# esteinig/scrubby

Hardware: AMD Instinct MI355X
Metric: reads/s depleted (2x150bp PE vs CHM13v2-sized reference), records classified per second (higher is better)
Workload: dtype u64/i32 (f32 in the chain gap penalty)

## Files before the change

scrubby_amd/csrc/sh_classify.hip:

```cpp
#include "sh_common.h"
#include "sh_wave.h"
#include "sh_merge4.h"
#include "sh_sketch.h"
#include "sh_chain.h"
#include "sh_long.h"
#include "sh_ctx_layout.h"
#include <algorithm>
#include <chrono>
#include <memory>

#define SH_SPLIT ((sh_status)-2)
#define K1_LIST_CAP 8
#define K2_CAP 32
#define DP_SMALL_CAP 32
#define SORT_LDS_A 512
#define SORT_LDS_B 2048
#define SORT_LDS_C 4096
#define N_SORT_CLS 6
#define SORT_CLS_GIANT 5
#define GT 2048u
#define LOCUS_N0 1024u
#define LOCUS_N1 4096u
#define LOCUS_MAX_N 65535u
#define LOCUS_RUN_MAX 16

__device__ inline uint32_t lane_id() { return threadIdx.x & 63; }

struct Counters {
    uint32_t n_small, n_resketch, n_big[2], n_big_defer[2], n_defer, n_small2;
    uint32_t n_big_total, pad1;
    uint32_t n_sort[N_SORT_CLS], n_giant_tiles, n_giant_passes;
    uint32_t expand_ticket, lc_ticket;
    uint32_t top_ticket[N_SORT_CLS];
    uint32_t sort_ticket[N_SORT_CLS];
    uint32_t n_long_segs, pad2;
    uint32_t ext_reason[8];
    uint32_t lext_exact_direct, lext_pad_d;
    uint32_t lc_why[16]; unsigned long long lc_anchors[16];
    uint32_t ext_overflow, ext_n_list, ext_ticket, ext_regions, ext_dropped, ext_n_redo, ext_n_list2, ext_ticket2, ext_n_redo2, ext_ticket3, ext_n_unres, ext_ticket_unres, ext_n_unres_in, ext_pad8;
    uint32_t ext_n_recs[SINK_SHARDS]; unsigned long long ext_n_anch[SINK_SHARDS];
    uint32_t lext_n_exact2, lext_ticket_exact2;
    uint32_t lext_hist[64]; uint32_t lext_ticket_g, lext_pad3; uint32_t lext_n_big, lext_ticket_big, lext_n_big2, lext_ticket_big2, lext_ticket_b, lext_pad2, lext_rechained, lext_rmq_tie, lext_err_read, lext_unresolved, lext_err_code, lext_pad;
    unsigned long long lext_clk[LR_NCLK], lext_d[8], lext_slow, lext_kernel_sum;
    uint32_t n_cl[4], cl_ticket, cl_ticket3;
    uint32_t n_leg_reason[4];
    uint32_t pair_mid[4];
    unsigned long long arena_cursor, anchor_cursor;
    unsigned long long cl_tot[4], cl_anchor_tot[4], cl_dbg[10], pf_dbg[16];
    unsigned long long sort_tot[N_SORT_CLS + 1], sort_anchor_tot[N_SORT_CLS + 1];
    unsigned long long sh_mini[64], sh_anchors[64];
    uint32_t sh_host[64], sh_clusters[64], sh_pair[64];
    uint32_t sh_late[64], sh_deferred[64];
    uint32_t sh_pf_reads[64], sh_pf_dirty[64], sh_top[64];
    uint32_t sh_lemma[64];
    uint32_t n_locus[3], locus_ticket[3], lr_n_fb, lr_locus_reads; unsigned long long lr_locus_in, lr_locus_kept;
    uint32_t lr_fb_why[8], lr_fb_had, lr_pad, lr_probe_why[8];
    uint32_t lext_n_unres, lext_ticket_unres, lext_n_unres_in, lext_pad4, lext_n_exact, lext_ticket_exact, lext_rmq_open, lext_pad5;
    unsigned long long ext_clk[8], ext_diag[8]; uint32_t ext_hist[24];
    unsigned long long lext_slow2, lext_slow3, lext_slow_part[4], lext_sum_part[4], lext_clk_big[LR_NCLK], lext_d_big[8], lext_phase_max[LR_NCLK];
    uint32_t lext_started, lext_t0_done;
    unsigned long long stage_cursor;
};
#define SHARD() ((blockIdx.x + (blockIdx.x >> 6)) & 63)

struct WaveAlloc {
    uint32_t cur = 0, end = 0;
    __device__ inline uint32_t take(uint32_t *counter, uint32_t n, uint32_t chunk, uint32_t &lo, uint32_t &hi)
    {
        lo = hi = 0;
        if (cur + n > end) {
            lo = cur; hi = end;
            const uint32_t want = n > chunk ? n : chunk;
            uint32_t base = 0;
            if (lane_id() == 0) base = atomicAdd(counter, want);
            base = (uint32_t)__builtin_amdgcn_readfirstlane((int)base);
            cur = base; end = base + want;
        }
        const uint32_t r = cur;
        cur += n;
        return r;
    }
};

__device__ inline uint32_t prefix_popc(uint64_t mask)
{
    return __builtin_amdgcn_mbcnt_hi((uint32_t)(mask >> 32), __builtin_amdgcn_mbcnt_lo((uint32_t)mask, 0u));
}
__device__ inline uint32_t wave_append(uint32_t *counter, bool pred)
{
    uint64_t mask = __ballot(pred);
    if (mask == 0) return ~0u;
    uint32_t base = 0;
    uint32_t leader = __ffsll((unsigned long long)mask) - 1;
    if (lane_id() == leader) base = atomicAdd(counter, (uint32_t)__popcll(mask));
    base = (uint32_t)wave_bcast((int32_t)base, (int)leader);
    return pred ? base + prefix_popc(mask) : ~0u;
}

__device__ inline void write_trace(sh_trace *tr, uint64_t r, int32_t n_mini, int32_t n_seed, int32_t n_anchor, int32_t rep_len,
                                   int32_t rechained, int32_t n_chain, int32_t best, int32_t flag)
{
    if (!tr) return;
    int4 *p = (int4 *)(tr + r);
    p[0] = make_int4(n_mini, n_seed, n_anchor, rep_len);
    p[1] = make_int4(rechained, n_chain, best, flag);
    p[2] = make_int4(0, 0, 0, 0);
}

struct K1Args {
    const uint8_t *bases; const uint64_t *offsets; uint64_t n_reads, n_bases;
    const uint4 *slots; uint32_t lg_slots; int32_t k;
    uint4 *records; uint32_t seed_cap;
    uint32_t *k1info; uint8_t *flags; sh_trace *trace;
    uint32_t *work_small, *work_resketch, *work_big; Counters *ctr;
// ... 1472 lines not shown
        if (in_lds) {
            uint64_t x = lane < n_a ? e_x[lane] : ~0ull;
            uint32_t q = lane < n_a ? e_q[lane] : 0u;
            uint64_t xp = wave_shr1_u64(x, 0ull);
            if (__ballot(lane > 0 && lane < n_a && x < xp) != 0) {
                wave_rank_sort(x, q, n_a, lane);
                __syncthreads();
                if (lane < n_a) { e_x[lane] = x; e_q[lane] = q; }
                __syncthreads();
            }
            int32_t n_u = 0, best = 0;
            bool lemma_done = false;
            if (a.t_mode && P.ext_lemma) {
                BestChain bc{};
                chain_sorted<false>(e_x, e_q, e_f, e_pt, n_a, lane, 64, qlen, P, nullptr, BigList{e_bstart, e_blen, &e_bcount, 8}, n_u, best, n_clusters,
                                    nullptr, nullptr, nullptr, r, nullptr, &bc, region_hash(qlen), -1, TandemQ{recb, n_seed, 1u, qlen, LONG ? 1u : info >> 31});
                unsigned long long zmax = bc.n ? bc.z : 0ull;
                zmax = wave_all_max_u64(zmax);
                const uint64_t holders = __ballot(bc.n > 0 && bc.z == zmax);
                const uint64_t any = __ballot(bc.n > 0);
                bool ok = false;
                if (any == 0) ok = true;
                else if (__popcll(holders) == 1) {
                    int32_t code = 0;
                    MidReq mid{0, 0, 0, 0, 0};
                    if (bc.n > 0 && bc.z == zmax && !bc.tie) {
                        SliceStore S{(const uint64_t *)&e_x[bc.base], (const uint32_t *)&e_q[bc.base], e_f + bc.base, e_pt + 2 * (size_t)bc.base};
                        code = chain_lemma(S, bc.zi, bc.end_i, P, (uint32_t)(S.X(bc.zi) >> 32), mid);
                    }
                    const bool mid_ok = resolve_mid_wave(code == 2, mid, a.BC.bases + a.offsets[r], qlen, a.BC, P);
                    ok = __ballot(code == 1 || (code == 2 && mid_ok)) != 0;
                }
                lemma_done = ok;
                if (ok && any != 0) ++n_lemma;
                if (!ok) { n_u = 0; best = 0; __syncthreads(); }
            }
            if (!lemma_done)
            chain_sorted<false>(e_x, e_q, e_f, e_pt, n_a, lane, 64, qlen, P, nullptr, BigList{e_bstart, e_blen, &e_bcount, 8}, n_u, best, n_clusters,
                                nullptr, nullptr, a.emit ? &sink_l : nullptr, r, nullptr);
            n_u = wave_all_add(n_u); best = wave_all_max(best);
            if (lane == 0) { a.B.acc_nu[w] = n_u; a.B.acc_best[w] = best; }
            if ((a.dbg & DBG_STATS) && lane == 0) { atomicAdd(&a.ctr->sort_tot[N_SORT_CLS], 1ull); atomicAdd(&a.ctr->sort_anchor_tot[N_SORT_CLS], (unsigned long long)n_a); }
            __syncthreads();
        } else if (to_stage) {
            const int lc = n_a <= LOCUS_N0 ? 0 : (n_a <= LOCUS_N1 ? 1 : 2);
            if (lane == 0) { const uint32_t li = atomicAdd(&a.ctr->n_locus[lc], 1u); SortItem it{w, n_a, (uint32_t)qlen, 0, off}; a.locus_items[lc][li] = it; }
        } else {
            uint32_t lo, hi;
            const uint32_t si = al_sort[cls].take(&a.ctr->n_sort[cls], 1, cls <= 1 ? 32u : (cls <= 3 ? 8u : 1u), lo, hi);
            SortItem *const items = a.B.tabs->sort_items[cls];
            for (uint32_t i = lo + lane; i < hi; i += 64) items[i].n = 0;
            if (lane == 0) { SortItem it{w, n_a, (uint32_t)qlen, late ? late_item(r, n_seed) : 0u, off}; items[si] = it; }
            n_late += late;
            if ((a.dbg & DBG_STATS) && lane == 0) { atomicAdd(&a.ctr->sort_tot[cls], 1ull); atomicAdd(&a.ctr->sort_anchor_tot[cls], (unsigned long long)n_a); }
        }
    }
    for (int cls = 0; cls < N_SORT_CLS; ++cls)
        for (uint32_t i = al_sort[cls].cur + lane; i < al_sort[cls].end; i += 64) a.B.tabs->sort_items[cls][i].n = 0;
    if (lane == 0 && anchors_wave) atomicAdd(&a.ctr->sh_anchors[SHARD()], anchors_wave);
    n_clusters = wave_sum_u32(n_clusters);
    if (lane == 0 && n_clusters) atomicAdd(&a.ctr->sh_clusters[SHARD()], n_clusters);
    if (lane == 0 && n_pair) atomicAdd(&a.ctr->sh_pair[SHARD()], n_pair);
    if (lane == 0 && n_late && !a.quiet) atomicAdd(&a.ctr->sh_late[SHARD()], n_late);
    if (lane == 0 && n_deferred) atomicAdd(&a.ctr->sh_deferred[SHARD()], n_deferred);
    if (lane == 0 && n_lemma) atomicAdd(&a.ctr->sh_lemma[SHARD()], n_lemma);
}

template <int LG>
__global__ __launch_bounds__(256) void k_lr_locus(K3Args a, int lc)
{
    __shared__ uint32_t s_tab[1u << (LG - 1)];
    __shared__ uint32_t s_it, s_w[4][4], s_wcnt[4], s_off[3];
    __shared__ uint32_t s_keep[(LOCUS_MAX_N + 1) / 32 + 8];
    const uint32_t tid = threadIdx.x, lane = tid & 63, wave = tid >> 6;
    const uint32_t n_items = a.ctr->n_locus[lc];
    const int sh = a.locus_shift;
    const uint32_t min_cnt = (uint32_t)(a.P.min_cnt > 1 ? a.P.min_cnt : 1);
    auto bin_of = [&](uint64_t x) -> uint64_t { return (x >> 32) << 24 | (uint64_t)((uint32_t)x >> sh); };
    auto slot = [&](uint64_t id) -> uint32_t { return (uint32_t)((id * 0x9E3779B97F4A7C15ull) >> (64 - LG)); };
    auto cnt_of = [&](uint64_t id) -> uint32_t { const uint32_t h = slot(id); return (s_tab[h >> 1] >> ((h & 1u) << 4)) & 0xffffu; };
    auto block_max = [&](uint32_t v, int k) -> uint32_t {
        v = wave_all_max_u32(v);
        if (lane == 0) s_w[k][wave] = v;
        __syncthreads();
        return max(max(s_w[k][0], s_w[k][1]), max(s_w[k][2], s_w[k][3]));
    };
    unsigned long long st_in = 0, st_kept = 0; uint32_t st_reads = 0;
    for (;;) {
        if (tid == 0) s_it = atomicAdd(&a.ctr->locus_ticket[lc], 1u);
        __syncthreads();
        const uint32_t it = s_it;
        __syncthreads();
        if (it >= n_items) break;
        const SortItem si = a.locus_items[lc][it];
        const uint32_t n = si.n;
        const uint64_t *gx = a.stage_x + si.off; const uint32_t *gq = a.stage_q + si.off;
        for (uint32_t i = tid; i < (1u << (LG - 1)); i += 256) s_tab[i] = 0;
        __syncthreads();
        for (uint32_t i = tid; i < n; i += 256) { const uint32_t h = slot(bin_of(gx[i])); atomicAdd(&s_tab[h >> 1], 1u << ((h & 1u) << 4)); }
        __syncthreads();
        auto bound_of = [&](uint64_t x) -> uint32_t {
            const uint64_t id = bin_of(x);
            uint32_t vr = cnt_of(id);
            int len = 1; bool inf = false;
            for (int d = 1;; ++d) { if (d > LOCUS_RUN_MAX) { inf = true; break; } const uint32_t c = cnt_of(id - (uint64_t)d); if (!c) break; vr += c; ++len; }
            if (!inf) for (int d = 1;; ++d) { if (d > LOCUS_RUN_MAX) { inf = true; break; } const uint32_t c = cnt_of(id + (uint64_t)d); if (!c) break; vr += c; ++len; }
            return (inf || len > LOCUS_RUN_MAX) ? 0x7fffffffu : vr;
// ... 210 lines not shown
            if (hit) { store_read_result(a, si.w, tid == 0 ? 1 : 0, 0, n_cl0, s_red); __syncthreads(); continue; }
            for (uint32_t i = tid; i < n; i += NTHR) { s_x[0][i] = gx[i]; s_q[0][i] = gq[i]; }
            if (tid == 0) s_found = 0;
            __syncthreads();
        }
        const bool fl = block_merge_sort(&s_x[0][0], &s_q[0][0], &s_x[1][0], &s_q[1][0], n);
        uint64_t *rx = fl ? s_x[1] : s_x[0]; uint32_t *rq = fl ? s_q[1] : s_q[0];
        int32_t *f = (int32_t *)(fl ? s_q[0] : s_q[1]), *pt = (int32_t *)(fl ? s_x[0] : s_x[1]);
        int32_t n_u = 0, best = 0; uint32_t n_cl = 0;
        const bool to_q = CLS >= 1 && a.cl_lds && n > 256u;
        const GlobalQ clq{a.B.tabs->cl_items, a.B.tabs->cl_cap, a.ctr->n_cl, si.w, 1u, si.off};
        if (!(a.dbg & DBG_NO_CHAIN_LDS))
        chain_sorted<false>(rx, rq, f, pt, n, tid, NTHR, (int32_t)si.qlen, a.P, a.flag_only ? &s_found : nullptr,
                            BigList{s_bstart, s_blen, &s_bcount, NMAX / 7 + 1}, n_u, best, n_cl, to_q ? &clq : nullptr, nullptr,
                            a.emit ? &a.sink : nullptr, a.B.meta[si.w].r, a.emit ? a.B.hz + si.off : nullptr,
                            nullptr, 0u, -1, TandemQ{nullptr, 0u, 1u, 0, 0u}, use_pf ? &s_pf : nullptr, nullptr, (a.dbg & DBG_STATS) ? a.ctr->pf_dbg : nullptr,
                            (a.quiet || (a.emit && a.sink.best && !(a.dbg & DBG_NO_TOPBT))) ? nullptr : a.ctr->sh_pf_reads,
                            to_q ? a.B.bx + si.off : nullptr, to_q ? a.B.bq + si.off : nullptr, 256u);
        store_read_result(a, si.w, n_u, best, n_cl, s_red);
        __syncthreads();
    }
}


__device__ inline uint32_t giant_lf(uint32_t fanin) { return fanin == 4 ? 2u : 1u; }
__device__ inline uint32_t giant_passes(uint32_t n, uint32_t fanin) { return m4_passes(n, GT, giant_lf(fanin)); }

template <class PX, class PQ>
__device__ inline bool fix_dirty_clusters(PX x, PQ q, int32_t *f, int32_t *pt, uint32_t n, int32_t qlen, const ChainParams &P, uint32_t tid, uint32_t nthr, const ParFillLds &L,
                                          uint32_t max_len, int32_t *s_left)
{
    const uint32_t wave = tid >> 6, n_wave = nthr >> 6, lane = tid & 63;
    const int32_t nd = L.n_dirty;
    if (tid == 0) *s_left = 0;
    __syncthreads();
    for (int32_t d = (int32_t)wave; d < nd; d += (int32_t)n_wave) {
        uint32_t c = L.dirty[d];
        while (!((uint32_t)q[c] >> 31)) --c;
        uint32_t e = c + 1;
        while (e < n && !((uint32_t)q[e] >> 31)) ++e;
        if (e - c > max_len) { if (lane == 0) *s_left = 1; continue; }
        int32_t mine = 0;
        if (lane == 0) mine = atomicCAS(&pt[2 * (size_t)c + 1], (int32_t)PF_DIRTY, (int32_t)PF_DEAD) == (int32_t)PF_DIRTY ? 1 : 0;
        mine = __builtin_amdgcn_readfirstlane(mine);
        if (!mine) continue;
        SliceStore S{(const uint64_t *)&x[c], (const uint32_t *)&q[c], f + c, pt + 2 * (size_t)c};
        chain_dp_wave(S, (int)(e - c), qlen, P, lane);
        for (uint32_t i = c + lane; i < e; i += 64) { const int32_t pv = pt[2 * (size_t)i]; if (pv >= 0) pt[2 * (size_t)i] = pv + (int32_t)c; pt[2 * (size_t)i + 1] = 0; }
    }
    __syncthreads();
    return *s_left == 0;
}

template <int NMAX, int CLS, int NTHR>
__global__ __launch_bounds__(NTHR) void k_sort_top(K3Args a)
{
    __shared__ uint64_t s_x[2][NMAX];
    __shared__ uint32_t s_q[2][NMAX];
    __shared__ ParFillLds s_pf;
    __shared__ long long s_top[18];
    __shared__ uint32_t s_cf[TOPBT_MAX], s_ci[TOPBT_MAX], s_it;
    __shared__ int32_t s_cn, s_red[2];
    const ChainSink sink_l = a.sink; const ChainParams P_l = a.P;
    const uint32_t tid = threadIdx.x;
    const uint32_t n_items = a.ctr->n_sort[CLS];
    unsigned long long *const dbg = (a.dbg & DBG_STATS) ? a.ctr->pf_dbg : nullptr;
    for (;;) {
        if (tid == 0) s_it = atomicAdd(&a.ctr->top_ticket[CLS], 1u);
        __syncthreads();
        const uint32_t it = s_it;
        __syncthreads();
        if (it >= n_items) break;
        const SortItem si = a.B.sort_items[CLS][it];
        const uint32_t n = si.n;
        if (n == 0) continue;
        const int32_t qlen = (int32_t)si.qlen;
        const uint64_t *gx = a.B.ax + si.off; const uint32_t *gq = a.B.aq + si.off;
        if (late_class(CLS) && si.pad) late_anchors(si.pad, qlen, 0u, n, &s_x[0][0], &s_q[0][0], tid, NTHR, (uint32_t *)&s_x[1][0]);
        else for (uint32_t i = tid; i < n; i += NTHR) { s_x[0][i] = gx[i]; s_q[0][i] = gq[i]; }
        __syncthreads();
        const bool fl = block_merge_sort(&s_x[0][0], &s_q[0][0], &s_x[1][0], &s_q[1][0], n);
        uint64_t *rx = fl ? s_x[1] : s_x[0]; uint32_t *rq = fl ? s_q[1] : s_q[0];
        int32_t *f = (int32_t *)(fl ? s_q[0] : s_q[1]), *pt = (int32_t *)(fl ? s_x[0] : s_x[1]);
        const uint32_t mdx = chain_max_dist_x(P_l, qlen);
        uint32_t starts = 0;
        for (uint32_t i = tid; i < n; i += NTHR) {
            bool start = i == 0;
            if (!start) { const uint64_t xi = rx[i], xp = rx[i - 1]; start = (uint32_t)(xi >> 32) != (uint32_t)(xp >> 32) || (uint32_t)xi - (uint32_t)xp > mdx; }
            if (start) { rq[i] |= 0x80000000u; ++starts; }
        }
        __syncthreads();
        if (!par_fill_block(rx, rq, f, pt, n, qlen, P_l, tid, NTHR, s_pf)) { if (dbg && tid == 0) atomicAdd(&dbg[1], 1ull); continue; }
        if (tid == 0 && !a.quiet) { atomicAdd(&a.ctr->sh_pf_reads[SHARD()], 1u); if (s_pf.n_dirty) atomicAdd(&a.ctr->sh_pf_dirty[SHARD()], (uint32_t)s_pf.n_dirty); }
        fix_dirty_clusters(rx, rq, f, pt, n, qlen, P_l, tid, NTHR, s_pf, 0xffffffffu, &s_cn);
        SliceStore S{(const uint64_t *)rx, (const uint32_t *)rq, f, pt};
        const uint32_t read = a.B.meta[si.w].r;
        const StoreEmit<SliceStore> em{&sink_l, &S, read, 0u, tid == 0, P_l.k, region_hash(qlen), qlen, nullptr};
        int32_t n_u = 0, best = 0;
        const bool settled = backtrack_block_top(S, (int32_t)n, P_l, n_u, best, em, sink_l, read, tid, NTHR, s_top, s_cf, s_ci, &s_cn, (uint32_t)a.top_max, dbg);
        if (!settled) continue;
        store_read_result(a, si.w, tid == 0 ? n_u : 0, best, starts, s_red);
        if (tid == 0) { a.B.sort_items[CLS][it].n = 0; if (!a.quiet) atomicAdd(&a.ctr->sh_top[SHARD()], 1u); }
        __syncthreads();
    }
}

#define GIANT_TOP_NTHR 512
static_assert(sizeof(ParFillLds) + sizeof(PfTile) + sizeof(long long[18]) + 2 * sizeof(uint32_t[TOPBT_MAX]) + 4 * sizeof(uint32_t) + 64 <= PFT_LDS_BUDGET, "k_giant_top: three blocks per CU");
__global__ __launch_bounds__(GIANT_TOP_NTHR, 6) void k_giant_top(K3Args a)
{
    __shared__ ParFillLds s_pf;
    __shared__ PfTile s_tile;
    __shared__ long long s_top[18];
    __shared__ uint32_t s_cf[TOPBT_MAX], s_ci[TOPBT_MAX], s_it;
    __shared__ int32_t s_cn, s_red[2];
    const ChainSink sink_l = a.sink; const ChainParams P_l = a.P;
    const uint32_t tid = threadIdx.x, nthr = blockDim.x;
    const uint32_t n_items = a.ctr->n_sort[SORT_CLS_GIANT];
    unsigned long long *const dbg = (a.dbg & DBG_STATS) ? a.ctr->pf_dbg : nullptr;
    const bool top = a.emit && sink_l.best != nullptr && !(a.dbg & DBG_NO_TOPBT);
    for (;;) {
        if (tid == 0) s_it = atomicAdd(&a.ctr->top_ticket[SORT_CLS_GIANT], 1u);
        __syncthreads();
        const uint32_t it = s_it;
        __syncthreads();
        if (it >= n_items) break;
        const uint32_t slot = a.B.giant_order[it];
        const SortItem si = a.B.sort_items[SORT_CLS_GIANT][slot];
// ... 1245 lines not shown
    hipLaunchKernelGGL(k_long_scan, dim3(1), dim3(1024), 0, s, a, 1);
    hipLaunchKernelGGL(k_long_scan, dim3(512), dim3(1024), 0, s, a, 2);
    hipLaunchKernelGGL((k_long_sketch<W, true>), dim3(256 * 8), dim3(256), 0, s, a);
    hipLaunchKernelGGL(k_long_probe, dim3(256 * 16), dim3(64), 0, s, a);
}

static sh_status ensure_side_streams(sh_ctx *c, int first, int last)
{
    for (int i = first; i <= last; ++i)
        if (!c->sx[i]) SH_HIP(c->own.stream(c->sx[i], hipStreamNonBlocking));
    return SH_OK;
}

__global__ void k_spin(unsigned long long ticks)
{
    const unsigned long long t0 = wall_clock64();
    while (wall_clock64() - t0 < ticks) __builtin_amdgcn_s_sleep(8);
}

static sh_status pick_side_streams(sh_ctx *c, hipStream_t s)
{
    if (c->side_probed_done && c->side_probed == s) return SH_OK;
    sh_status es = ensure_side_streams(c, 0, 2);
    if (es != SH_OK) return es;
    if (c->cs.side_pick >= 0) { c->side_pick[0] = (int)c->cs.side_pick & 255; c->side_pick[1] = (int)c->cs.side_pick >> 8; c->side_probed = s; c->side_probed_done = true; return SH_OK; }
    DevEvent ev_t0, ev_t1, ev_e;
    SH_HIP(ev_t0.create()); SH_HIP(ev_t1.create()); SH_HIP(ev_e.create(hipEventDisableTiming));
    float ms[3] = {1e9f, 1e9f, 1e9f};
    for (int i = 0; i < 3; ++i) {
        float rep[3] = {0, 0, 0};
        for (int k = 0; k < 3; ++k) {
            SH_HIP(hipStreamSynchronize(s));
            SH_HIP(hipEventRecord(ev_t0.e, s));
            SH_HIP(hipStreamWaitEvent(c->sx[i], ev_t0.e, 0));
            hipLaunchKernelGGL(k_spin, dim3(1), dim3(64), 0, s, 20000ull);
            hipLaunchKernelGGL(k_spin, dim3(1), dim3(64), 0, c->sx[i], 20000ull);
            SH_HIP(hipEventRecord(ev_e.e, c->sx[i]));
            SH_HIP(hipStreamWaitEvent(s, ev_e.e, 0));
            SH_HIP(hipEventRecord(ev_t1.e, s));
            SH_HIP(hipEventSynchronize(ev_t1.e));
            SH_HIP(hipEventElapsedTime(&rep[k], ev_t0.e, ev_t1.e));
        }
        std::sort(rep, rep + 3);
        ms[i] = rep[1];
    }
    int ord[3] = {0, 1, 2};
    std::sort(ord, ord + 3, [&](int a, int b) { return ms[a] < ms[b]; });
    c->side_pick[0] = ord[0]; c->side_pick[1] = ord[1];
    c->side_probed = s; c->side_probed_done = true;
    if (c->cs.dbg_set) fprintf(stderr, "[dbg] side streams beside the caller's: %.2f %.2f %.2f ms for two 0.2-ms kernels; giants on %d, follower on %d\n", ms[0], ms[1], ms[2], c->side_pick[0], c->side_pick[1]);
    return SH_OK;
}

static sh_status big_pass(sh_ctx *c, K3Args k, uint32_t grid, hipStream_t s)
{
    Counters *ctr = c->d_ctr;
    SH_HIP(hipMemsetAsync(&ctr->anchor_cursor, 0, 8, s));
    SH_HIP(hipMemsetAsync(&ctr->n_sort[0], 0, 4 * N_SORT_CLS, s));
    SH_HIP(hipMemsetAsync(&ctr->sort_ticket[0], 0, 4 * N_SORT_CLS, s));
    SH_HIP(hipMemsetAsync(&ctr->expand_ticket, 0, 4, s));
    SH_HIP(hipMemsetAsync(&ctr->n_cl[0], 0, 4 * 6, s));
    if (k.flag_only && k.P.flag_stop != INT32_MAX && !(k.dbg & DBG_NO_GROUP_PROBE)) k.late = 0;
    if (k.locus) { SH_HIP(hipMemsetAsync(&ctr->n_locus[0], 0, 4 * 6, s)); SH_HIP(hipMemsetAsync(&ctr->stage_cursor, 0, 8, s)); }
    if (k.seed_off) hipLaunchKernelGGL(k_expand<true>, dim3(grid * 3), dim3(64), 0, s, k);
    else hipLaunchKernelGGL(k_expand<false>, dim3(grid * 3), dim3(64), 0, s, k);
    if (k.locus && k.seed_off) {
        hipLaunchKernelGGL(k_lr_locus<12>, dim3(256 * 8), dim3(256), 0, s, k, 0);
        hipLaunchKernelGGL(k_lr_locus<14>, dim3(256 * 5), dim3(256), 0, s, k, 1);
        hipLaunchKernelGGL(k_lr_locus<15>, dim3(256 * 2), dim3(256), 0, s, k, 2);
    }
    const int64_t side_env = c->cs.side;
    const bool gp = k.flag_only && k.P.flag_stop != INT32_MAX && !(k.dbg & DBG_NO_GROUP_PROBE);
    const bool side = side_env == 1 || (side_env < 0 && !gp && c->cur_reads <= 3000000ull);
    if (side) { sh_status es = ensure_side_streams(c, 0, 2); if (es != SH_OK) return es; }
    hipStream_t s0 = side ? c->sx[0] : s, s1 = side ? c->sx[1] : s, g = side ? c->sx[2] : s;
    const bool use_pf = (k.emit || !k.flag_only) && !(k.dbg & DBG_NO_PARFILL);
    const bool use_top = use_pf && k.emit && k.sink.best != nullptr && !(k.dbg & DBG_NO_TOPBT);
    if (use_pf) SH_HIP(hipMemsetAsync(&ctr->top_ticket[0], 0, 4 * N_SORT_CLS, s));
    if (side) {
        SH_HIP(hipEventRecord(c->evx[0], s));
        for (int i = 0; i < 3; ++i) SH_HIP(hipStreamWaitEvent(c->sx[i], c->evx[0], 0));
    }
    if (gp) {
        hipLaunchKernelGGL(k_group_probe, dim3(256 * 3), dim3(256), 0, s, k, 4);
        hipLaunchKernelGGL(k_group_probe, dim3(256 * 3), dim3(256), 0, s, k, (int)SORT_CLS_GIANT);
    }
    const bool aside = use_top && !side && !k.cl_lds && side_env != 0;
    hipStream_t sa = s;
    if (aside) {
        sh_status ps = pick_side_streams(c, s);
        if (ps != SH_OK) return ps;
        sa = c->sx[c->side_pick[0]];
    }
    auto lds_stream = [&](int cls, hipStream_t own, hipStream_t &out) -> sh_status {
        out = own;
        if (!aside) return SH_OK;
        SH_HIP(hipEventRecord(c->evx[8 + cls], own));
        SH_HIP(hipStreamWaitEvent(sa, c->evx[8 + cls], 0));
        out = sa;
        return SH_OK;
    };
    hipStream_t sl = s;
    sh_status ls = SH_OK;
    if (use_top) hipLaunchKernelGGL((k_sort_top<256, 0, 64>), dim3(grid * 2), dim3(64), 0, s, k);
    if ((ls = lds_stream(0, s, sl)) != SH_OK) return ls;
    hipLaunchKernelGGL((k_sort_lds<256, 0, 64>), dim3(grid * 2), dim3(64), 0, sl, k);
    if (use_top) hipLaunchKernelGGL((k_sort_top<SORT_LDS_A, 1, 128>), dim3(grid * 2), dim3(128), 0, s, k);
    if ((ls = lds_stream(1, s, sl)) != SH_OK) return ls;
    hipLaunchKernelGGL((k_sort_lds<SORT_LDS_A, 1, 128>), dim3(grid * 2), dim3(128), 0, sl, k);
    if (use_top) hipLaunchKernelGGL((k_sort_top<1024, 2, 256>), dim3(256 * 6), dim3(256), 0, s0, k);
    if ((ls = lds_stream(2, s0, sl)) != SH_OK) return ls;
    hipLaunchKernelGGL((k_sort_lds<1024, 2, 256>), dim3(256 * 6), dim3(256), 0, sl, k);
    if (use_top) hipLaunchKernelGGL((k_sort_top<SORT_LDS_B, 3, 256>), dim3(256 * 3), dim3(256), 0, s0, k);
    if ((ls = lds_stream(3, s0, sl)) != SH_OK) return ls;
    hipLaunchKernelGGL((k_sort_lds<SORT_LDS_B, 3, 256>), dim3(256 * 3), dim3(256), 0, sl, k);
    if (use_top) hipLaunchKernelGGL((k_sort_top<SORT_LDS_C, 4, 512>), dim3(256), dim3(512), 0, s1, k);
    if ((ls = lds_stream(4, s1, sl)) != SH_OK) return ls;
    hipLaunchKernelGGL((k_sort_lds<SORT_LDS_C, 4, 512>), dim3(256), dim3(512), 0, sl, k);
    hipLaunchKernelGGL(k_giant_scan, dim3(1), dim3(1024), 0, g, k);
    hipLaunchKernelGGL(k_giant_chunksort, dim3(256 * 3), dim3(256), 0, g, k);
    for (uint32_t pass = 0; pass < (k.giant_fanin == 4 ? 4u : 8u); ++pass) {
        hipLaunchKernelGGL(k_giant_split, dim3(256), dim3(256), 0, g, k, pass);
        hipLaunchKernelGGL(k_giant_merge4, dim3(256 * 6), dim3(256), 0, g, k, pass);
    }
    const bool two_phase = k.t_mode && k.sink.best != nullptr;
    if (use_pf) hipLaunchKernelGGL(k_giant_top, dim3(1024), dim3(GIANT_TOP_NTHR), 0, g, k);
    hipLaunchKernelGGL(k_giant_chain, dim3(1024), dim3(512), 0, g, k, two_phase ? 0 : -1);
    if (side && k.cl_lds) {
        SH_HIP(hipEventRecord(c->evx[1], c->sx[0])); SH_HIP(hipStreamWaitEvent(g, c->evx[1], 0));
        SH_HIP(hipEventRecord(c->evx[2], c->sx[1])); SH_HIP(hipStreamWaitEvent(g, c->evx[2], 0));
        SH_HIP(hipEventRecord(c->evx[6], s)); SH_HIP(hipStreamWaitEvent(g, c->evx[6], 0));
    }
    if (!(k.dbg & DBG_NO_CLUSTER_DP)) hipLaunchKernelGGL(k_cluster_dp, dim3(256 * 7), dim3(256), 0, g, k);
    if (two_phase) {
        SH_HIP(hipMemsetAsync(&ctr->sort_ticket[SORT_CLS_GIANT], 0, 4, g));
        hipLaunchKernelGGL(k_giant_chain, dim3(1024), dim3(512), 0, g, k, 1);
    }
    if (side) for (int i = 0; i < 3; ++i) { SH_HIP(hipEventRecord(c->evx[1 + i], c->sx[i])); SH_HIP(hipStreamWaitEvent(s, c->evx[1 + i], 0)); }
    if (aside) { SH_HIP(hipEventRecord(c->evx[13], sa)); SH_HIP(hipStreamWaitEvent(s, c->evx[13], 0)); }
    hipLaunchKernelGGL(k_finalize, dim3(grid), dim3(256), 0, s, k);
    return SH_OK;
}

static sh_status launch_front_end(sh_ctx *c, const uint8_t *d_bases, const uint64_t *d_offsets, uint64_t n_reads, uint64_t n_bases,
                                  uint8_t *d_flags, sh_trace *d_trace, hipStream_t s)
{
    const sh_index *idx = c->idx;
    const uint32_t n_tiles = (uint32_t)((n_reads + 63) / 64);
    if (c->use_k1) {
        K1Args a{};
        a.bases = d_bases; a.offsets = d_offsets; a.n_reads = n_reads; a.n_bases = n_bases;
        a.slots = (const uint4 *)idx->d_slots; a.lg_slots = idx->lg_slots; a.k = idx->k;
        a.records = c->d_records; a.seed_cap = c->seed_cap;
        a.k1info = c->d_k1info; a.flags = d_flags; a.trace = d_trace;
        a.work_small = c->d_work_small; a.work_resketch = c->d_work_resketch; a.work_big = c->d_big[0][0]; a.ctr = c->d_ctr;
        a.lds_words = c->lds_words; a.mid_occ = c->P.mid_occ;
        a.q_occ_max = (c->P.q_occ_frac > 0.0f && c->P.mid_occ > 0) ? (uint32_t)c->P.mid_occ : UINT32_MAX;
        size_t lds = (((size_t)K1_LIST_CAP * 64 * 8 + ((size_t)c->lds_words + 2) * 6 + 7) & ~(size_t)7) + 64 * 8;
        switch (idx->w) {
        case 5: launch_k1<5>(a, n_tiles, lds, s); break;
        case 10: launch_k1<10>(a, n_tiles, lds, s); break;
        case 11: launch_k1<11>(a, n_tiles, lds, s); break;
        case 19: launch_k1<19>(a, n_tiles, lds, s); break;
        default: sh_set_error("unsupported w"); return SH_ERR_BAD_ARG;
        }
    } else if (c->use_long) {
        LongArgs a{};
        a.bases = d_bases; a.offsets = d_offsets; a.n_reads = n_reads; a.n_bases = n_bases;
        a.slots = (const uint4 *)idx->d_slots; a.lg_slots = idx->lg_slots; a.k = idx->k;
        a.seg_base = c->d_seg_base; a.seg_cnt = c->d_seg_cnt; a.seg_off = c->d_seg_off; a.scan_tot = c->d_scan_tot;
        a.mz_hash = c->d_mz_hash; a.mz_y = c->d_mz_y; a.mz_cap = c->mz_cap; a.lrec = c->d_lrec; a.seed_off = c->d_seed_off;
        a.k1info = c->d_k1info; a.flags = d_flags; a.trace = d_trace;
        a.work_big = c->d_big[0][0]; a.work_resketch = c->d_work_resketch; a.ctr = c->d_ctr;
        a.mid_occ = c->P.mid_occ;
        a.q_occ_max = (c->P.q_occ_frac > 0.0f && c->P.mid_occ > 0) ? (uint32_t)c->P.mid_occ : UINT32_MAX;
        a.q_occ_frac = c->P.q_occ_frac;
        a.n_segs_out = &c->d_ctr->n_long_segs; a.max_segs = (uint32_t)std::min<uint64_t>(c->max_segs, UINT32_MAX);
        switch (idx->w) {
        case 5: launch_long<5>(a, s); break;
        case 10: launch_long<10>(a, s); break;
        case 11: launch_long<11>(a, s); break;
        case 19: launch_long<19>(a, s); break;
        default: sh_set_error("unsupported w"); return SH_ERR_BAD_ARG;
        }
    } else {
        hipLaunchKernelGGL(k_route_all, dim3((uint32_t)((n_reads + 255) / 256)), dim3(256), 0, s, n_reads, c->d_work_resketch, c->d_ctr);
    }
    return SH_OK;
}

#define SH_TRY(call) do { const sh_status st_ = (call); if (st_ != SH_OK) return st_; } while (0)

static sh_status read_counters(sh_ctx *c, hipStream_t s)
{
    SH_HIP(hipMemcpyAsync(c->h_ctr, c->d_ctr, sizeof(Counters), hipMemcpyDeviceToHost, s));
    SH_HIP(hipStreamSynchronize(s));
    SH_HIP(hipGetLastError());
    return SH_OK;
}

static void print_repeat_pass(const Counters &h, int iter)
{
    fprintf(stderr, "[dbg] iter %d resketch %u reasons %u %u %u pair tests between two singletons (dbg) %u segs %u big %u/%u defer %u/%u\n", iter, h.n_resketch, h.n_leg_reason[0], h.n_leg_reason[1], h.n_leg_reason[2], h.n_leg_reason[3], h.n_long_segs, h.n_big[0], h.n_big[1], h.n_big_defer[0], h.n_big_defer[1]);
    fprintf(stderr, "[dbg] clusters chained by k_cluster_dp by class: %llu %llu %llu %llu, their anchors %llu %llu %llu %llu\n", h.cl_tot[0], h.cl_tot[1], h.cl_tot[2], h.cl_tot[3], h.cl_anchor_tot[0], h.cl_anchor_tot[1], h.cl_anchor_tot[2], h.cl_anchor_tot[3]);
    fprintf(stderr, "[dbg] reads (anchors) by sort class: <=64 %llu (%llu), <=256 %llu (%llu), <=512 %llu (%llu), <=1024 %llu (%llu), <=2048 %llu (%llu), <=4096 %llu (%llu), giant %llu (%llu)\n", h.sort_tot[6], h.sort_anchor_tot[6], h.sort_tot[0], h.sort_anchor_tot[0], h.sort_tot[1], h.sort_anchor_tot[1], h.sort_tot[2], h.sort_anchor_tot[2], h.sort_tot[3], h.sort_anchor_tot[3], h.sort_tot[4], h.sort_anchor_tot[4], h.sort_tot[5], h.sort_anchor_tot[5]);
    fprintf(stderr, "[dbg] pair pass mode 2: premises hold but too many bases outside the k-mers: LDS path %u, of which the middle check decided %u; repeat path %u, decided %u\n", h.pair_mid[0], h.pair_mid[1], h.pair_mid[2], h.pair_mid[3]);
    static const char *const lc_name[] = {"tried", "no singleton", "a seed above mid_occ", "singletons apart", "window grew / too many", "K size", "no margin over U_out", "lemma / no chain / tie", "decided", "decided, seeds filtered", "seeds not 2..64"};
    fprintf(stderr, "[dbg] local-cluster shortcut, reads (anchors the occurrence filter admits):");
    for (int i = 0; i <= LC_N_SEED; ++i) fprintf(stderr, "%s %s %u (%llu)", i ? "," : "", lc_name[i], h.lc_why[i], h.lc_anchors[i]);
    fprintf(stderr, "\n");
    fprintf(stderr, "[dbg] ring DP: chunks in window %llu, beyond %llu, far rescans %llu; clusters %llu (anchors %llu), with a max_skip break %llu (anchors %llu), widest window %llu, anchors of clusters with a window > 64: %llu, > 128: %llu\n", h.cl_dbg[0], h.cl_dbg[1], h.cl_dbg[2], h.cl_dbg[3], h.cl_dbg[6], h.cl_dbg[4], h.cl_dbg[5], h.cl_dbg[7], h.cl_dbg[8], h.cl_dbg[9]);
    fprintf(stderr, "[dbg] parallel fill: reads done %llu (anchors %llu), not applicable %llu (anchors %llu), dirty anchors %llu; k_cluster_dp clusters prefilled %llu, sequential %llu (anchors %llu); read-level backtracks tried %llu, candidates listed %llu, given up (too many) %llu, chains visited %llu\n", h.pf_dbg[0], h.pf_dbg[3], h.pf_dbg[1], h.pf_dbg[4], h.pf_dbg[2], h.pf_dbg[5], h.pf_dbg[6], h.pf_dbg[7], h.pf_dbg[8], h.pf_dbg[11], h.pf_dbg[12], h.pf_dbg[10]);
}

static void print_first_round(const Counters &h, bool locus, uint32_t n_fb)
{
    if (locus) fprintf(stderr, "[dbg] anchors by locus: %u reads thinned out (%llu of %llu anchors kept); %u reads redone with every anchor (one chain and more possible %u, short read %u, top score within reach of what was left out %u, no chain after the join %u, probe undecided %u, no probe %u, no chain among the anchors kept %u)\n",
                       h.lr_locus_reads, h.lr_locus_kept, h.lr_locus_in, n_fb, h.lr_fb_why[0], h.lr_fb_why[1], h.lr_fb_why[2], h.lr_fb_why[3], h.lr_fb_why[4], h.lr_fb_why[5], h.lr_fb_why[6]);
    fprintf(stderr, "[dbg] probes that gave up (first round): region %u, window %u, filling over 4 M cells %u, direction bytes %u, z-drop / empty %u, CIGAR room %u, no proof within six fillings %u\n",
            h.lr_probe_why[1], h.lr_probe_why[2], h.lr_probe_why[3], h.lr_probe_why[4], h.lr_probe_why[5], h.lr_probe_why[6], h.lr_probe_why[7]);
}

static void print_long_stage(const Counters &h, const Chunk &ch, const ChainSink &sink)
{
    fprintf(stderr, "[dbg] long-read extension stage: %u reads with chains, %u re-chained (RMQ), %u with tied RMQ priorities, %u needed the large scratch, %u regions aligned, %u reads dropped\n",
            ch.ext_list, h.lext_rechained, h.lext_rmq_tie, ch.n_big_a, h.ext_regions, h.ext_dropped);
    unsigned long long tot = 0, mr = 0, ma = 0, sr = 0, sa = 0;
    for (int i = 0; i < LR_NCLK; ++i) tot += h.lext_clk[i];
    fprintf(stderr, "[dbg] long-read extension stage, share of wave time: gather %.1f  rmq-sort %.1f  rmq-fill %.1f  backtrack+compact %.1f  gen_regs %.1f  parent/select %.1f  squeeze %.1f  region set-up %.1f  ksw %.1f  z-drop test %.1f  update_extra %.1f  staging %.1f %%  (total %.1f wave-s at 100 MHz)\n",
            100. * h.lext_clk[0] / (tot + 1), 100. * h.lext_clk[1] / (tot + 1), 100. * h.lext_clk[2] / (tot + 1), 100. * h.lext_clk[3] / (tot + 1), 100. * h.lext_clk[4] / (tot + 1), 100. * h.lext_clk[5] / (tot + 1),
            100. * h.lext_clk[6] / (tot + 1), 100. * h.lext_clk[7] / (tot + 1), 100. * h.lext_clk[8] / (tot + 1), 100. * h.lext_clk[9] / (tot + 1), 100. * h.lext_clk[10] / (tot + 1), 100. * h.lext_clk[11] / (tot + 1), tot / 1e8);
    fprintf(stderr, "[dbg] RMQ: %llu reads, %llu anchors (largest read %llu), per anchor: %.2f ring blocks, %.3f trips behind the ring with %.2f old blocks, list length %.1f, %.2f inner chunks\n",
            h.lext_d[6], h.lext_d[0], h.lext_d[7], (double)h.lext_d[1] / (h.lext_d[0] + 1), (double)h.lext_d[2] / (h.lext_d[0] + 1),
            (double)h.lext_d[3] / (h.lext_d[0] + 1), (double)h.lext_d[4] / (h.lext_d[0] + 1), (double)h.lext_d[5] / (h.lext_d[0] + 1));
    fprintf(stderr, "[dbg] chains kernel: slowest read %.1f ms (%llu chains after the long join; read %llu of the chunk, %llu bases), all reads %.1f wave-ms\n", (h.lext_slow >> 24) / 1e5, h.lext_slow & 0xffffff,
            h.lext_slow3 & 0xffffffffull, h.lext_slow2 & 0xffffffffull, h.lext_kernel_sum / 1e5);
    { unsigned long long tb = 0; for (int i = 0; i < LR_NCLK; ++i) tb += h.lext_clk_big[i];
      fprintf(stderr, "[dbg] regions kernel, second size: gen_regs %.1f  parent/select %.1f  squeeze %.1f  set-up %.1f  ksw %.1f  z-drop %.1f  update_extra %.1f  staging %.1f %% of %.1f wave-s\n", 100. * h.lext_clk_big[4] / (tb + 1), 100. * h.lext_clk_big[5] / (tb + 1), 100. * h.lext_clk_big[6] / (tb + 1), 100. * h.lext_clk_big[7] / (tb + 1), 100. * h.lext_clk_big[8] / (tb + 1), 100. * h.lext_clk_big[9] / (tb + 1), 100. * h.lext_clk_big[10] / (tb + 1), 100. * h.lext_clk_big[11] / (tb + 1), tb / 1e8); }
    { unsigned long long tg = h.lext_clk_big[0] + h.lext_clk_big[1] + h.lext_clk_big[2] + h.lext_clk_big[3];
      fprintf(stderr, "[dbg] giants rmq-fill sections (wave-s): insert %.2f  trim %.2f  query %.2f  tally %.2f  score+inner %.2f\n", h.lext_clk_big[4] / 1e8, h.lext_clk_big[5] / 1e8, h.lext_clk_big[6] / 1e8, h.lext_clk_big[7] / 1e8, h.lext_clk_big[8] / 1e8);
      fprintf(stderr, "[dbg] all rmq-fill sections (wave-s): insert %.2f  trim %.2f  query %.2f  tally %.2f  score+inner %.2f\n", h.lext_clk[4] / 1e8, h.lext_clk[5] / 1e8, h.lext_clk[6] / 1e8, h.lext_clk[7] / 1e8, h.lext_clk[8] / 1e8);
      fprintf(stderr, "[dbg] chains kernel, the giants: gather %.1f  rmq-sort %.1f  rmq-fill %.1f  backtrack+compact %.1f %% of %.2f wave-s\n", 100. * h.lext_clk_big[0] / (tg + 1), 100. * h.lext_clk_big[1] / (tg + 1), 100. * h.lext_clk_big[2] / (tg + 1), 100. * h.lext_clk_big[3] / (tg + 1), tg / 1e8); }
    { const unsigned long long *dd = h.lext_d_big;
      fprintf(stderr, "[dbg] RMQ, the giants: %llu reads, %llu anchors (largest read %llu), per anchor: %.2f ring blocks, %.3f trips behind the ring with %.2f old blocks, list length %.1f, %.2f inner chunks\n",
              dd[6], dd[0], dd[7], (double)dd[1] / (dd[0] + 1), (double)dd[2] / (dd[0] + 1), (double)dd[3] / (dd[0] + 1), (double)dd[4] / (dd[0] + 1), (double)dd[5] / (dd[0] + 1)); }
    fprintf(stderr, "[dbg] regions kernel, second size: slowest read %.1f ms (%llu bases), all reads %.1f wave-ms\n", (h.lext_slow_part[3] >> 32) / 1e5, h.lext_slow_part[3] & 0xffffffffull, h.lext_sum_part[3] / 1e5);
    fprintf(stderr, "[dbg] regions kernel, second size, largest per-read time of each step (ms): gen_regs %.1f  parent/select %.1f  squeeze %.1f  set-up %.1f  ksw %.1f  z-drop %.1f  update_extra %.1f  staging %.1f\n", h.lext_phase_max[4] / 1e5, h.lext_phase_max[5] / 1e5, h.lext_phase_max[6] / 1e5, h.lext_phase_max[7] / 1e5, h.lext_phase_max[8] / 1e5, h.lext_phase_max[9] / 1e5, h.lext_phase_max[10] / 1e5, h.lext_phase_max[11] / 1e5);
    for (int pp = 0; pp < 3; ++pp) fprintf(stderr, "[dbg] chains kernel, part %d (0 lists of later passes, 1 all but the giants, 2 the giants): slowest read %.1f ms, all reads %.1f wave-ms\n", pp, (h.lext_slow_part[pp] >> 32) / 1e5, h.lext_sum_part[pp] / 1e5);
    for (int i = 0; i < SINK_SHARDS; ++i) { sr += h.ext_n_recs[i]; sa += h.ext_n_anch[i]; mr = std::max<unsigned long long>(mr, h.ext_n_recs[i]); ma = std::max<unsigned long long>(ma, h.ext_n_anch[i]); }
    fprintf(stderr, "[dbg] chain hand-over: %llu chains, %llu anchors; fullest shard %llu / %u chains, %llu / %llu anchors\n", sr, sa, mr, sink.cap_recs, ma, sink.cap_anch);
}

static void print_align_top(const Counters &h, uint32_t waves_top)
{
    unsigned long long tot = 0;
    for (int i = 0; i < ACLK_N; ++i) tot += h.ext_clk[i];
    fprintf(stderr, "[dbg] k_regs_align_top, %u waves: ksw fill %.1f  ksw backtrack %.1f  staging %.1f  lane-0 walks %.1f  other %.1f %% of %.3f wave-s; %u reads, %u ksw_extd2 calls (%u with T16 <= 256, Q16 <= 336 and the exact maximum)\n",
            waves_top, 100. * h.ext_clk[0] / (tot + 1), 100. * h.ext_clk[1] / (tot + 1), 100. * h.ext_clk[2] / (tot + 1), 100. * h.ext_clk[3] / (tot + 1), 100. * h.ext_clk[4] / (tot + 1), tot / 1e8, h.ext_hist[22], h.ext_hist[20], h.ext_hist[21]);
// ... 767 lines not shown
```

Measured before the change: 122.3 million.

## Split large-class sort_top kernels into LDS-sized rungs for higher occupancy

Sort classes 3 and 4 each become two kernel instantiations (rungs) with smaller NMAX, so reads with fewer anchors run in kernels that use less LDS and fit more resident blocks per CU. Each rung scans the same item table through its own ticket and skips items outside its (nmin, nmax] range. Grid sizes come from an occupancy query so the grid matches the resident blocks. The cost is that every rung reads the whole table, which adds extra ticket atomics and item loads, plus extra kernel launches. Debug histograms of anchor counts in classes 3 and 4 are added as well.

```diff
diff --git a/scrubby_amd/csrc/sh_classify.hip b/scrubby_amd/csrc/sh_classify.hip
--- a/scrubby_amd/csrc/sh_classify.hip
+++ b/scrubby_amd/csrc/sh_classify.hip
@@ -1,6 +1,7 @@
 #include "sh_common.h"
 #include "sh_wave.h"
 #include "sh_merge4.h"
+#include "sh_sort_rungs.h"
 #include "sh_sketch.h"
 #include "sh_chain.h"
 #include "sh_long.h"
@@ -18,6 +19,7 @@
 #define SORT_LDS_C 4096
 #define N_SORT_CLS 6
 #define SORT_CLS_GIANT 5
+#define RUNG_HIST_BINS ((SORT_LDS_C - 1024) / 64)
 #define GT 2048u
 #define LOCUS_N0 1024u
 #define LOCUS_N1 4096u
@@ -32,6 +34,7 @@
     uint32_t n_sort[N_SORT_CLS], n_giant_tiles, n_giant_passes;
     uint32_t expand_ticket, lc_ticket;
     uint32_t top_ticket[N_SORT_CLS];
+    uint32_t rung_ticket[SORT_N_RUNGS + (SORT_N_RUNGS & 1)];
     uint32_t sort_ticket[N_SORT_CLS];
     uint32_t n_long_segs, pad2;
     uint32_t ext_reason[8];
@@ -60,6 +63,7 @@
     unsigned long long lext_slow2, lext_slow3, lext_slow_part[4], lext_sum_part[4], lext_clk_big[LR_NCLK], lext_d_big[8], lext_phase_max[LR_NCLK];
     uint32_t lext_started, lext_t0_done;
     unsigned long long stage_cursor;
+    unsigned long long rung_hist_reads[2][RUNG_HIST_BINS], rung_hist_anchors[2][RUNG_HIST_BINS];
 };
 #define SHARD() ((blockIdx.x + (blockIdx.x >> 6)) & 63)
 
@@ -1638,7 +1642,10 @@
             for (uint32_t i = lo + lane; i < hi; i += 64) items[i].n = 0;
             if (lane == 0) { SortItem it{w, n_a, (uint32_t)qlen, late ? late_item(r, n_seed) : 0u, off}; items[si] = it; }
             n_late += late;
-            if ((a.dbg & DBG_STATS) && lane == 0) { atomicAdd(&a.ctr->sort_tot[cls], 1ull); atomicAdd(&a.ctr->sort_anchor_tot[cls], (unsigned long long)n_a); }
+            if ((a.dbg & DBG_STATS) && lane == 0) {
+                atomicAdd(&a.ctr->sort_tot[cls], 1ull); atomicAdd(&a.ctr->sort_anchor_tot[cls], (unsigned long long)n_a);
+                if (cls == 3 || cls == 4) { const uint32_t bin = (n_a - 1025u) >> 6; atomicAdd(&a.ctr->rung_hist_reads[a.pass & 1][bin], 1ull); atomicAdd(&a.ctr->rung_hist_anchors[a.pass & 1][bin], (unsigned long long)n_a); }
+            }
         }
     }
     for (int cls = 0; cls < N_SORT_CLS; ++cls)
@@ -1955,9 +1962,11 @@
     return *s_left == 0;
 }
 
-template <int NMAX, int CLS, int NTHR>
+template <int NMIN, int NMAX, int CLS, int NTHR>
 __global__ __launch_bounds__(NTHR) void k_sort_top(K3Args a)
 {
+    constexpr int RUNG = sort_rung_of(NMAX);
+    static_assert(RUNG >= 0 && SORT_RUNGS[RUNG].cls == CLS && SORT_RUNGS[RUNG].nmin == NMIN && SORT_RUNGS[RUNG].nmax == NMAX && SORT_RUNGS[RUNG].nthr == NTHR, "k_sort_top is instantiated from SORT_RUNGS");
     __shared__ uint64_t s_x[2][NMAX];
     __shared__ uint32_t s_q[2][NMAX];
     __shared__ ParFillLds s_pf;
@@ -1969,7 +1978,7 @@
     const uint32_t n_items = a.ctr->n_sort[CLS];
     unsigned long long *const dbg = (a.dbg & DBG_STATS) ? a.ctr->pf_dbg : nullptr;
     for (;;) {
-        if (tid == 0) s_it = atomicAdd(&a.ctr->top_ticket[CLS], 1u);
+        if (tid == 0) s_it = atomicAdd(&a.ctr->rung_ticket[RUNG], 1u);
         __syncthreads();
         const uint32_t it = s_it;
         __syncthreads();
@@ -1977,6 +1986,11 @@
         const SortItem si = a.B.sort_items[CLS][it];
         const uint32_t n = si.n;
         if (n == 0) continue;
+        if constexpr (!sort_rung_alone(RUNG)) {
+            uint32_t nn = n;
+            asm volatile("" : "+v"(nn));
+            if (nn <= (uint32_t)NMIN || nn > (uint32_t)NMAX) continue;
+        }
         const int32_t qlen = (int32_t)si.qlen;
         const uint64_t *gx = a.B.ax + si.off; const uint32_t *gq = a.B.aq + si.off;
         if (late_class(CLS) && si.pad) late_anchors(si.pad, qlen, 0u, n, &s_x[0][0], &s_q[0][0], tid, NTHR, (uint32_t *)&s_x[1][0]);
@@ -3328,6 +3342,40 @@
     return SH_OK;
 }
 
+struct RungGrids { uint32_t per_cu[SORT_N_RUNGS], blocks[SORT_N_RUNGS]; bool ok; };
+
+template <int I = 0>
+static void rung_grids_fill(RungGrids &g)
+{
+    if constexpr (I < SORT_N_RUNGS) {
+        if constexpr (SORT_RUNGS[I].cls >= 3) {
+            int per_cu = 0;
+            const auto kern = &k_sort_top<SORT_RUNGS[I].nmin, SORT_RUNGS[I].nmax, SORT_RUNGS[I].cls, SORT_RUNGS[I].nthr>;
+            if (hipOccupancyMaxActiveBlocksPerMultiprocessor(&per_cu, kern, SORT_RUNGS[I].nthr, 0) != hipSuccess || per_cu <= 0) { g.ok = false; per_cu = 0; }
+            g.per_cu[I] = (uint32_t)per_cu; g.blocks[I] = 256u * (uint32_t)per_cu;
+        }
+        rung_grids_fill<I + 1>(g);
+    }
+}
+
+static RungGrids rung_grids()
+{
+    RungGrids g{};
+    g.ok = true;
+    rung_grids_fill(g);
+    return g;
+}
+
+template <int CLS, int I = 0>
+static void launch_rungs(const RungGrids &g, hipStream_t s, const K3Args &k)
+{
+    if constexpr (I < SORT_N_RUNGS) {
+        if constexpr (SORT_RUNGS[I].cls == CLS)
+            hipLaunchKernelGGL((k_sort_top<SORT_RUNGS[I].nmin, SORT_RUNGS[I].nmax, SORT_RUNGS[I].cls, SORT_RUNGS[I].nthr>), dim3(g.blocks[I]), dim3(SORT_RUNGS[I].nthr), 0, s, k);
+        launch_rungs<CLS, I + 1>(g, s, k);
+    }
+}
+
 static sh_status big_pass(sh_ctx *c, K3Args k, uint32_t grid, hipStream_t s)
 {
     Counters *ctr = c->d_ctr;
@@ -3353,6 +3401,14 @@
     const bool use_pf = (k.emit || !k.flag_only) && !(k.dbg & DBG_NO_PARFILL);
     const bool use_top = use_pf && k.emit && k.sink.best != nullptr && !(k.dbg & DBG_NO_TOPBT);
     if (use_pf) SH_HIP(hipMemsetAsync(&ctr->top_ticket[0], 0, 4 * N_SORT_CLS, s));
+    if (use_top) SH_HIP(hipMemsetAsync(&ctr->rung_ticket[0], 0, 4 * SORT_N_RUNGS, s));
+    static const RungGrids rungs = rung_grids();
+    SH_CHECK(!use_top || rungs.ok, SH_ERR_HIP, "k_sort_top: a rung has no resident block");
+    if ((k.dbg & DBG_STATS) && use_top && k.pass == 0) {
+        fprintf(stderr, "[dbg] k_sort_top rungs of tables 3 and 4, resident blocks per CU (cut for):");
+        for (int i = 0; i < SORT_N_RUNGS; ++i) if (SORT_RUNGS[i].cls >= 3) fprintf(stderr, " (%d, %d] %u (%d)", SORT_RUNGS[i].nmin, SORT_RUNGS[i].nmax, rungs.per_cu[i], SORT_RUNGS[i].blocks);
+        fprintf(stderr, "\n");
+    }
     if (side) {
         SH_HIP(hipEventRecord(c->evx[0], s));
         for (int i = 0; i < 3; ++i) SH_HIP(hipStreamWaitEvent(c->sx[i], c->evx[0], 0));
@@ -3378,19 +3434,19 @@
     };
     hipStream_t sl = s;
     sh_status ls = SH_OK;
-    if (use_top) hipLaunchKernelGGL((k_sort_top<256, 0, 64>), dim3(grid * 2), dim3(64), 0, s, k);
+    if (use_top) hipLaunchKernelGGL((k_sort_top<64, 256, 0, 64>), dim3(grid * 2), dim3(64), 0, s, k);
     if ((ls = lds_stream(0, s, sl)) != SH_OK) return ls;
     hipLaunchKernelGGL((k_sort_lds<256, 0, 64>), dim3(grid * 2), dim3(64), 0, sl, k);
-    if (use_top) hipLaunchKernelGGL((k_sort_top<SORT_LDS_A, 1, 128>), dim3(grid * 2), dim3(128), 0, s, k);
+    if (use_top) hipLaunchKernelGGL((k_sort_top<256, SORT_LDS_A, 1, 128>), dim3(grid * 2), dim3(128), 0, s, k);
     if ((ls = lds_stream(1, s, sl)) != SH_OK) return ls;
     hipLaunchKernelGGL((k_sort_lds<SORT_LDS_A, 1, 128>), dim3(grid * 2), dim3(128), 0, sl, k);
-    if (use_top) hipLaunchKernelGGL((k_sort_top<1024, 2, 256>), dim3(256 * 6), dim3(256), 0, s0, k);
+    if (use_top) hipLaunchKernelGGL((k_sort_top<SORT_LDS_A, 1024, 2, 256>), dim3(256 * 6), dim3(256), 0, s0, k);
     if ((ls = lds_stream(2, s0, sl)) != SH_OK) return ls;
     hipLaunchKernelGGL((k_sort_lds<1024, 2, 256>), dim3(256 * 6), dim3(256), 0, sl, k);
-    if (use_top) hipLaunchKernelGGL((k_sort_top<SORT_LDS_B, 3, 256>), dim3(256 * 3), dim3(256), 0, s0, k);
+    if (use_top) launch_rungs<3>(rungs, s0, k);
     if ((ls = lds_stream(3, s0, sl)) != SH_OK) return ls;
     hipLaunchKernelGGL((k_sort_lds<SORT_LDS_B, 3, 256>), dim3(256 * 3), dim3(256), 0, sl, k);
-    if (use_top) hipLaunchKernelGGL((k_sort_top<SORT_LDS_C, 4, 512>), dim3(256), dim3(512), 0, s1, k);
+    if (use_top) launch_rungs<4>(rungs, s1, k);
     if ((ls = lds_stream(4, s1, sl)) != SH_OK) return ls;
     hipLaunchKernelGGL((k_sort_lds<SORT_LDS_C, 4, 512>), dim3(256), dim3(512), 0, sl, k);
     hipLaunchKernelGGL(k_giant_scan, dim3(1), dim3(1024), 0, g, k);
@@ -3480,6 +3536,11 @@
     fprintf(stderr, "[dbg] iter %d resketch %u reasons %u %u %u pair tests between two singletons (dbg) %u segs %u big %u/%u defer %u/%u\n", iter, h.n_resketch, h.n_leg_reason[0], h.n_leg_reason[1], h.n_leg_reason[2], h.n_leg_reason[3], h.n_long_segs, h.n_big[0], h.n_big[1], h.n_big_defer[0], h.n_big_defer[1]);
     fprintf(stderr, "[dbg] clusters chained by k_cluster_dp by class: %llu %llu %llu %llu, their anchors %llu %llu %llu %llu\n", h.cl_tot[0], h.cl_tot[1], h.cl_tot[2], h.cl_tot[3], h.cl_anchor_tot[0], h.cl_anchor_tot[1], h.cl_anchor_tot[2], h.cl_anchor_tot[3]);
     fprintf(stderr, "[dbg] reads (anchors) by sort class: <=64 %llu (%llu), <=256 %llu (%llu), <=512 %llu (%llu), <=1024 %llu (%llu), <=2048 %llu (%llu), <=4096 %llu (%llu), giant %llu (%llu)\n", h.sort_tot[6], h.sort_anchor_tot[6], h.sort_tot[0], h.sort_anchor_tot[0], h.sort_tot[1], h.sort_anchor_tot[1], h.sort_tot[2], h.sort_anchor_tot[2], h.sort_tot[3], h.sort_anchor_tot[3], h.sort_tot[4], h.sort_anchor_tot[4], h.sort_tot[5], h.sort_anchor_tot[5]);
+    for (int p = 0; p < 2; ++p) {
+        fprintf(stderr, "[dbg] tables 3 and 4, pass %d, reads (anchors) per 64-anchor bin from 1025:", p);
+        for (int b = 0; b < RUNG_HIST_BINS; ++b) fprintf(stderr, " %llu (%llu)", h.rung_hist_reads[p][b], h.rung_hist_anchors[p][b]);
+        fprintf(stderr, "\n");
+    }
     fprintf(stderr, "[dbg] pair pass mode 2: premises hold but too many bases outside the k-mers: LDS path %u, of which the middle check decided %u; repeat path %u, decided %u\n", h.pair_mid[0], h.pair_mid[1], h.pair_mid[2], h.pair_mid[3]);
     static const char *const lc_name[] = {"tried", "no singleton", "a seed above mid_occ", "singletons apart", "window grew / too many", "K size", "no margin over U_out", "lemma / no chain / tie", "decided", "decided, seeds filtered", "seeds not 2..64"};
     fprintf(stderr, "[dbg] local-cluster shortcut, reads (anchors the occurrence filter admits):");
diff --git a/scrubby_amd/csrc/sh_sort_rungs.h b/scrubby_amd/csrc/sh_sort_rungs.h
--- /dev/null
+++ b/scrubby_amd/csrc/sh_sort_rungs.h
@@ -0,0 +1,30 @@
+#pragma once
+#include <stdint.h>
+
+#define SORT_TOP_LDS_PER_ANCHOR 24
+#define SORT_TOP_LDS_FIXED 2160
+#define SORT_CU_LDS_BYTES (160 * 1024)
+#define SORT_LDS_GRANULE 1280
+
+struct SortRung { int cls, nmin, nmax, nthr, blocks; };
+
+constexpr SortRung SORT_RUNGS[] = {
+    {0, 64, 256, 64, 16},
+    {1, 256, 512, 128, 8},
+    {2, 512, 1024, 256, 6},
+    {3, 1024, 1600, 256, 4},
+    {3, 1600, 2048, 256, 3},
+    {4, 2048, 3264, 512, 2},
+    {4, 3264, 4096, 512, 1},
+};
+constexpr int SORT_N_RUNGS = (int)(sizeof(SORT_RUNGS) / sizeof(SORT_RUNGS[0]));
+
+constexpr int sort_rung_lds(int nmax) { return SORT_TOP_LDS_PER_ANCHOR * nmax + SORT_TOP_LDS_FIXED; }
+constexpr int sort_rung_lds_budget(int blocks) { return SORT_CU_LDS_BYTES / SORT_LDS_GRANULE / blocks * SORT_LDS_GRANULE; }
+constexpr int sort_rung_of(int n)
+{
+    for (int i = 0; i < SORT_N_RUNGS; ++i) if (SORT_RUNGS[i].nmin < n && n <= SORT_RUNGS[i].nmax) return i;
+    return -1;
+}
+constexpr bool sort_rung_last_of_table(int i) { return i + 1 == SORT_N_RUNGS || SORT_RUNGS[i + 1].cls != SORT_RUNGS[i].cls; }
+constexpr bool sort_rung_alone(int i) { return (i == 0 || SORT_RUNGS[i - 1].cls != SORT_RUNGS[i].cls) && sort_rung_last_of_table(i); }
```

Result: faster. 124.9 million, median of 6 (+2.1%).
